# kotakondo/Intent-MPC

Hardware: AMD Instinct MI355X
Metric: QP-solves/s + p50 solve latency, N=20 horizon, batch=65536, 1/2/4/8 MI355X (higher is better)
Workload: dtype f64

## Files before the change

intent-mpc_amd/csrc/impc_qp.hip:

```cpp
#include <hip/hip_runtime.h>
#include <hipcub/hipcub.hpp>

#include <algorithm>
#include <cstdio>
#include <cstring>
#include <memory>
#include <string>
#include <type_traits>
#include <vector>

#include "../../include/impc_qp.h"
#include "../../include/impc_select.h"
#include "../../include/impc_mpc.h"
#include "../../include/impc_fanout.h"
#include "../../include/impc_predict.h"
#include "../../include/impc_detect.h"
#include "../../include/impc_comm.h"
#include "../../include/impc_replan.h"
#include "lib_internal.hpp"
#include "mpc_qp_internal.hpp"
#include "admm_core.hpp"
#include "mpc_structure.hpp"
#include "mpc_wave.hpp"
#include "queue.hpp"
// ... 115 lines not shown
        double qj = IMPC_AT(wk.q, j);
        if (st.scaling > 0) {
            qj = IMPC_AT(wk.D, j) * qj;
            qj *= c;
        }
        IMPC_AT(wk.qs, j) = qj;
    }
}

__global__ __launch_bounds__(kBlock) void k_update_bounds(impc::DevSym sy, impc::DevWork wk, impc::DevSettings st,
                                                          int64_t B) {
    const int lane = blockIdx.x * kBlock + threadIdx.x;
    if (lane >= B) return;
    const int64_t S = wk.S;
    const double rho = IMPC_AT(wk.scal, impc::SC_RHO);
    int changed = 0;
    for (int32_t i = 0; i < sy.m; i++) {
        double li = impc::dmin(impc::dmax(IMPC_AT(wk.l, i), -impc::kInf), impc::kInf);
        double ui = impc::dmin(impc::dmax(IMPC_AT(wk.u, i), -impc::kInf), impc::kInf);
        if (st.scaling > 0) {
            li = IMPC_AT(wk.E, i) * li;
            ui = IMPC_AT(wk.E, i) * ui;
        }
        IMPC_AT(wk.ls, i) = li;
        IMPC_AT(wk.us, i) = ui;
        double t, r;
        if ((li < -impc::kInf * impc::kMinScaling) && (ui > impc::kInf * impc::kMinScaling)) {
            t = -1.0;
            r = impc::kRhoMin;
        } else if (ui - li < impc::kRhoTol) {
            t = 1.0;
            r = rho * impc::kRhoEqOverIneq;
        } else {
            t = 0.0;
            r = rho;
        }
        if (IMPC_AT(wk.ctype, i) != t) {
            IMPC_AT(wk.ctype, i) = t;
            IMPC_AT(wk.rho, i) = r;
            IMPC_AT(wk.rhoinv, i) = 1. / r;
            changed = 1;
        }
    }
    if (changed) {
        int bad = impc::assemble_and_factor(sy, wk, st, lane);
        if (bad) IMPC_AT(wk.scal, impc::SC_SETUP_ERR) = (double)IMPC_NONCVX_ERROR;
    }
    impc::refresh_v(sy, wk, lane);
}

#ifndef IMPC_LCOMB
#define IMPC_LCOMB 1
#endif
template <int NL>
struct GpuTeam {
    double *red;
    __device__ int lane() const { return (int)threadIdx.x; }
    __device__ static void wave_sync() {
        __builtin_amdgcn_fence(__ATOMIC_ACQ_REL, "wavefront");
        __builtin_amdgcn_wave_barrier();
    }
    __device__ void sync() {
        if constexpr (NL == 64) wave_sync();
        else __syncthreads();
    }
    __device__ static void wsync() { wave_sync(); }
    __device__ void lsync() { sync(); }
    __device__ double bcast(double v, int src) {
        int lo = __builtin_amdgcn_readlane(__double2loint(v), src);
        int hi = __builtin_amdgcn_readlane(__double2hiint(v), src);
        return __hiloint2double(hi, lo);
    }
    __device__ static double uniform(double v) {
        int lo = __builtin_amdgcn_readfirstlane(__double2loint(v));
        int hi = __builtin_amdgcn_readfirstlane(__double2hiint(v));
        return __hiloint2double(hi, lo);
    }
    __device__ double shfl(double v, int src) {
        const int addr = src << 2;
        int lo = __builtin_amdgcn_ds_bpermute(addr, __double2loint(v));
        int hi = __builtin_amdgcn_ds_bpermute(addr, __double2hiint(v));
        return __hiloint2double(hi, lo);
    }
    template <int CTRL>
    __device__ static double dpp(double v) {
        int lo = __builtin_amdgcn_mov_dpp(__double2loint(v), CTRL, 0xF, 0xF, true);
        int hi = __builtin_amdgcn_mov_dpp(__double2hiint(v), CTRL, 0xF, 0xF, true);
        return __hiloint2double(hi, lo);
    }
    template <bool ODD>
    __device__ static double mfma_step(double f, double c, double v) {
        const double d = __builtin_amdgcn_mfma_f64_4x4x4f64(f, v, c, 0, 0, 0);
        return d + dpp<ODD ? 0x128 : 0x141>(d);
    }
    __device__ double sum_contig8(double v) {
        v = v + dpp<0xB1>(v);
        v = v + dpp<0x4E>(v);
        v = v + dpp<0x141>(v);
        return v;
    }
    __device__ static double add_dup(double x, double y) {
        double r;
        asm("v_add_f64 %0, %1, %2" : "=v"(r) : "v"(x), "v"(y));
        return r;
    }
    template <bool P32, bool DUP>
    __device__ static double pair_sum2(double a, double b, double *dup) {
        const int al = __double2loint(a), ah = __double2hiint(a), bl = __double2loint(b), bh = __double2hiint(b);
        auto rl = P32 ? __builtin_amdgcn_permlane32_swap(al, bl, false, false)
                      : __builtin_amdgcn_permlane16_swap(al, bl, false, false);
        auto rh = P32 ? __builtin_amdgcn_permlane32_swap(ah, bh, false, false)
                      : __builtin_amdgcn_permlane16_swap(ah, bh, false, false);
        const double x = __hiloint2double(rh[0], rl[0]), y = __hiloint2double(rh[1], rl[1]);
        if (DUP) *dup = add_dup(x, y);
        return x + y;
    }
    __device__ double sum_stride8(double v) {
        const double d = dpp<0x128>(v);
        const double a = v + d, b = add_dup(v, d);
        double c2;
        const double c = pair_sum2<false, true>(a, b, &c2);
        return pair_sum2<true, false>(c, c2, nullptr);
    }
    __device__ static double xor4(double v) {
        const int lo = __builtin_amdgcn_ds_swizzle(__double2loint(v), (4 << 10) | 0x1F);
        const int hi = __builtin_amdgcn_ds_swizzle(__double2hiint(v), (4 << 10) | 0x1F);
        return __hiloint2double(hi, lo);
    }
    __device__ double max(double v) {
        double mv[1] = {v};
        reduce<1, 0>(mv, nullptr);
        return mv[0];
    }
    template <int K>
    __device__ void max_n(double (&v)[K]) {
        reduce<K, 0>(v, nullptr);
    }
    template <int KM, int KS>
    __device__ void max_sum_n(double (&mx)[KM], double (&sm)[KS]) {
        reduce<KM, KS>(mx, sm);
    }
    template <bool P32>
    __device__ static void swap64(double &x, double &y) {
        const int xl = __double2loint(x), xh = __double2hiint(x), yl = __double2loint(y), yh = __double2hiint(y);
        auto rl = P32 ? __builtin_amdgcn_permlane32_swap(xl, yl, false, false)
                      : __builtin_amdgcn_permlane16_swap(xl, yl, false, false);
        auto rh = P32 ? __builtin_amdgcn_permlane32_swap(xh, yh, false, false)
                      : __builtin_amdgcn_permlane16_swap(xh, yh, false, false);
        x = __hiloint2double(rh[0], rl[0]);
        y = __hiloint2double(rh[1], rl[1]);
    }
    template <int KM, int KS>
    __device__ void reduce(double (&mx)[KM], double *sm) {
        constexpr int K1 = (KM + 1) / 2, K2 = (K1 + 1) / 2, KT = KM + KS;
        static_assert(KT * (NL / 64) <= impc::kRedLen, "team reduction scratch (WaveLds RED_OFF)");
        auto vmax = [](double a, double b) { return b > a ? b : a; };
        double h[K1], q[K2];
        _Pragma("unroll") for (int k = 0; k < K1; k++) {
            double x = mx[k], y = k + K1 < KM ? mx[k + K1] : mx[k];
            swap64<true>(x, y);
            h[k] = vmax(x, y);
        }
        _Pragma("unroll") for (int k = 0; k < K2; k++) {
            double x = h[k], y = k + K2 < K1 ? h[k + K2] : h[k];
            swap64<false>(x, y);
            double t = vmax(x, y);
            t = vmax(t, dpp<0xB1>(t));
            t = vmax(t, dpp<0x4E>(t));
            t = vmax(t, dpp<0x141>(t));
            q[k] = vmax(t, dpp<0x128>(t));
        }
        _Pragma("unroll") for (int k = 0; k < KS; k++) sm[k] = wave_sum(sm[k]);
        const int w = (int)threadIdx.x >> 6, row = ((int)threadIdx.x >> 4) & 3;
        if ((threadIdx.x & 15) == 0) {
            _Pragma("unroll") for (int k = 0; k < K2; k++) {
                const int sub = (row & 1) * K2 + k, idx = (row >> 1) * K1 + sub;
                if (sub < K1 && idx < KM) red[w * KT + idx] = q[k];
            }
        }
        if ((threadIdx.x & 63) == 0) _Pragma("unroll") for (int k = 0; k < KS; k++) red[w * KT + KM + k] = sm[k];
        __syncthreads();
#if IMPC_LCOMB
        if constexpr (NL > 64) {
            static_assert(KT <= 64, "one lane per reduced value");
            const int l = (int)threadIdx.x & 63, k = l < KT ? l : 0;
            double r = red[k];
            for (int u = 1; u < NL / 64; u++) {
                const double o = red[u * KT + k];
                const double m = vmax(r, o), a = r + o;
                r = k < KM ? m : a;
            }
            _Pragma("unroll") for (int j = 0; j < KM; j++) mx[j] = bcast(r, j);
            _Pragma("unroll") for (int j = 0; j < KS; j++) sm[j] = bcast(r, KM + j);
            __syncthreads();
            return;
        }
#endif
        _Pragma("unroll") for (int k = 0; k < KM; k++) {
            double r = red[k];
            for (int u = 1; u < NL / 64; u++) r = vmax(r, red[u * KT + k]);
            mx[k] = r;
        }
        _Pragma("unroll") for (int k = 0; k < KS; k++) {
            double r = red[KM + k];
            for (int u = 1; u < NL / 64; u++) r = r + red[u * KT + KM + k];
            sm[k] = r;
        }
        __syncthreads();
    }
    __device__ double wave_sum(double v) {
        {
            const int lo = __double2loint(v), hi = __double2hiint(v);
            auto ql = __builtin_amdgcn_permlane32_swap(lo, lo, false, false);
            auto qh = __builtin_amdgcn_permlane32_swap(hi, hi, false, false);
            v = __hiloint2double(qh[0], ql[0]) + __hiloint2double(qh[1], ql[1]);
        }
        {
            const int lo = __double2loint(v), hi = __double2hiint(v);
            auto rl = __builtin_amdgcn_permlane16_swap(lo, lo, false, false);
            auto rh = __builtin_amdgcn_permlane16_swap(hi, hi, false, false);
            v = __hiloint2double(rh[0], rl[0]) + __hiloint2double(rh[1], rl[1]);
        }
        v = v + dpp<0x128>(v);
        v = v + xor4(v);
        v = v + dpp<0x4E>(v);
        v = v + dpp<0xB1>(v);
        return v;
    }
    __device__ double sum(double v) {
        v = wave_sum(v);
        v = bcast(v, 0);
        if (NL == 64) return v;
        if ((threadIdx.x & 63) == 0) red[threadIdx.x >> 6] = v;
        __syncthreads();
        double r = red[0];
        for (int w = 1; w < NL / 64; w++) r = r + red[w];
        __syncthreads();
        return r;
    }
};

struct GroupEntry {
    impc::WaveTables T;
    impc::WaveIO io;
    impc::DevSettings st;
    int64_t first;
    const int64_t *dcount;
};

template <int NL, int VS, int GS, int WPS, int WF, bool TIER>
__global__ __launch_bounds__(NL, WPS) void k_mpc_wave_group(const GroupEntry *__restrict__ g, int count,
                                                            int64_t total, unsigned *counter,
                                                            const uint32_t *__restrict__ ord, int devcnt) {
    extern __shared__ __attribute__((aligned(16))) double smem[];
    using LD = impc::WaveLds<NL, VS, GS>;
    GpuTeam<NL> wv{smem + LD::RED_OFF};
    __shared__ unsigned next;
    int cur = -1;
    if (devcnt) {
        int64_t t = 0;
        for (int e = 0; e < count; e++) {
            const int64_t c = g[e].dcount ? *g[e].dcount : g[e].io.B;
            t += c < g[e].io.B ? (c > 0 ? c : 0) : g[e].io.B;
        }
        total = t;
    }
    for (;;) {
        if (threadIdx.x == 0) next = atomicAdd(counter, 1u);
        __syncthreads();
        const unsigned pos = next;
        __syncthreads();
        if ((int64_t)pos >= total) break;
        const unsigned b = ord ? ord[pos] : pos;
        int e = 0;
        while (e + 1 < count && (int64_t)b >= g[e + 1].first) e++;
        if (e != cur) {
            impc::WaveQP<GpuTeam<NL>, NL, VS, GS, WF, TIER>::load_tables(wv, g[e].T, smem);
            cur = e;
        }
        impc::WaveQP<GpuTeam<NL>, NL, VS, GS, WF, TIER> qp(wv, g[e].T, g[e].io, g[e].st, smem);
        qp.solve((int64_t)b - g[e].first);
    }
}

}

struct impc_ctx_s {
    int device = 0;
    int num_cu = 256;
    hipStream_t stream = nullptr;
    double tick_s = 1e-8;
    struct GroupTable {
        GroupEntry *d = nullptr;
        int cap = 0;
        std::vector<GroupEntry> h;
        uint64_t used = 0;
    };
    std::vector<GroupTable> groups;
    uint64_t group_clock = 0;
    hipEvent_t ev_order = nullptr;
    std::vector<hipEvent_t> ev_pool, ev_pending;
    std::vector<hipEvent_t> timer_marks;
    std::vector<std::pair<uint64_t, impc_batch_s *>> pool;
};

static int h2d_sync(hipStream_t st, void *dst, const void *src, size_t bytes) {
    if (!bytes) return IMPC_OK;
    HIP_OK(hipMemcpyAsync(dst, src, bytes, hipMemcpyHostToDevice, st));
    HIP_OK(hipStreamSynchronize(st));
    return IMPC_OK;
}
static int fill0_sync(hipStream_t st, void *dst, size_t bytes) {
    if (!bytes) return IMPC_OK;
    HIP_OK(hipMemsetAsync(dst, 0, bytes, st));
    HIP_OK(hipStreamSynchronize(st));
    return IMPC_OK;
}
#define IMPC_TRY(expr)          \
    do {                        \
        int rc_ = (expr);       \
        if (rc_) return rc_;    \
    } while (0)

static int ctx_order_launch(impc_ctx ctx, hipStream_t st) {
    if (st == ctx->stream) return IMPC_OK;
    if (!ctx->ev_order) HIP_OK(hipEventCreateWithFlags(&ctx->ev_order, hipEventDisableTiming));
    HIP_OK(hipEventRecord(ctx->ev_order, ctx->stream));
    HIP_OK(hipStreamWaitEvent(st, ctx->ev_order, 0));
    return IMPC_OK;
}
static int ctx_order_after_all(impc_ctx ctx, hipStream_t st) {
    if (st != ctx->stream) IMPC_TRY(ctx_order_launch(ctx, st));
    for (hipEvent_t e : ctx->ev_pending) HIP_OK(hipStreamWaitEvent(st, e, 0));
// ... 1970 lines not shown
```

intent-mpc_amd/csrc/mpc_wave.hpp:

```cpp
#pragma once
#include <hip/hip_runtime.h>
#include <math.h>
#include <stdint.h>

#include "../../include/impc_qp.h"
#include "admm_core.hpp"
#include "mpc_structure.hpp"
#include "sweep_mfma_map.hpp"

namespace impc {

#define IMPC_WF __host__ __device__ __forceinline__

#ifndef IMPC_PRIO
#define IMPC_PRIO 2
#endif
#if IMPC_PRIO && defined(__HIP_DEVICE_COMPILE__)
#define IMPC_PRIO_UP() __builtin_amdgcn_s_setprio(IMPC_PRIO)
#define IMPC_PRIO_DOWN() __builtin_amdgcn_s_setprio(0)
#else
#define IMPC_PRIO_UP() ((void)0)
#define IMPC_PRIO_DOWN() ((void)0)
#endif
#ifndef IMPC_SWEEP_MFMA
// ... 48 lines not shown

struct WaveTables {
    int32_t n, m, mg, N, W, CG, nnzP, nnzA;
    const int32_t *var_orig, *var_pdiag, *var_boxrow, *var_boxpos;
    const int32_t *gen_row, *gen_col, *gen_pos, *colg, *term_ptr, *term;
    int32_t HS;
    const int32_t *col_hid;
    int32_t T1r;
    int32_t scal_lds;
};

struct WaveIO {
    int64_t B;
    const double *Px, *q, *Ax, *l, *u, *xws, *yws;
    int32_t has_ws;
    double *xo, *yo;
    double *scal;
    impc_info *info;
    unsigned long long *sec = nullptr;
    unsigned long long *qpt = nullptr;
    int32_t shared = 0;
    int64_t nvar = 0;
    const int32_t *vmap = nullptr;
    const double *Ax_var = nullptr;
    double *persist = nullptr;
    int32_t resume = 0, q_updated = 0;
    const double *tlim = nullptr;
    const double *q_scale = nullptr;
};

constexpr int kPersistHdr = 24;
constexpr int kPersistMaxScaling = 20;
IMPC_HD int64_t persist_stride(int n, int mg) { return kPersistHdr + 3 * (int64_t)n + 2 * (int64_t)mg; }

enum {
    kSecSetup, kSecFactor, kSecWarm, kSecRhs, kSecS1, kSecFwd, kSecS3, kSecBwd, kSecS5, kSecUpdate, kSecProducts,
    kSecChecks, kSecOutput, kSecFAsm, kSecFDense, kSecIters = 15, kSecCount = 16
};
#if defined(IMPC_SECTION_PROF) && defined(__HIP_DEVICE_COMPILE__)
#define IMPC_SEC_CLOCK() ((uint64_t)__builtin_amdgcn_s_memrealtime())
#define IMPC_SEC(X)                             \
    do {                                        \
        uint64_t t_ = IMPC_SEC_CLOCK();         \
        sec_acc[X] += t_ - sec_t0;              \
        sec_t0 = t_;                            \
    } while (0)
#define IMPC_SEC_START() (sec_t0 = IMPC_SEC_CLOCK())
#else
#define IMPC_SEC(X) ((void)0)
#define IMPC_SEC_START() ((void)0)
#endif

constexpr int kRedLen = 128;

template <int NL, int VS, int GS>
struct WaveLds {
    static constexpr int NMAX = NL * VS;
    static constexpr int WMAX = (NMAX + 5) / 13 - 1;
    static constexpr int WSPEC = NMAX <= 256 ? 19 : 39;
    static constexpr int WSPEC2 = NMAX <= 256 ? 0 : 29;
    static constexpr int NP = (NMAX + 48 > (779 + NMAX + 3) / 4) ? NMAX + 48 : (779 + NMAX + 3) / 4;
    static constexpr int F_OFF = 0;
    static constexpr int R_OFF = F_OFF + WMAX * 64;
    static constexpr int T_OFF = R_OFF + NP;
    static constexpr int E_OFF = T_OFF + NP;
    static constexpr int X_OFF = E_OFF + NP;
    static constexpr int RED_OFF = X_OFF + NP;
    static constexpr int JUNK_OFF = RED_OFF + kRedLen;
    static constexpr int GSLOT_OFF = JUNK_OFF + NL;
    static constexpr bool ONCHIP = VS == 1;
    static constexpr int VEC_N = 2 * NMAX + NL * GS;
    static constexpr int SCL_OFF = GSLOT_OFF + NL * GS;
    static constexpr int DLT_OFF = SCL_OFF + (ONCHIP ? VEC_N : 0);
    static constexpr int DLT_N = ONCHIP && GS > 2 ? NL * (GS - 2) : 0;
    static constexpr int P_OFF = DLT_OFF + DLT_N;
    static constexpr int CGM = 24;
    static constexpr int T1 = kProdTier1;
    static IMPC_WF int cg4(int CG) { return (CG + 3) & ~3; }
    static constexpr IMPC_WF int stride(int n) { return ((n + 63) & ~63) + 1; }
    static IMPC_WF int hsp(int HS) { return HS + 1; }
    static IMPC_WF int p_size(int CG, int n, int HS, int mg, int T1r) {
        const int c = T1r * stride(n) + (cg4(CG) > T1r ? (cg4(CG) - T1r) * hsp(HS) : 0), f = 5 * mg;
        return c > f ? c : f;
    }
    static IMPC_WF int p_size(const WaveTables &T) { return p_size(T.CG, T.n, T.HS, T.mg, T.T1r); }
    static constexpr int CHX = (VS == 1 && IMPC_CHUNK19) ? 448 : 0;
    static IMPC_WF int ch_off(const WaveTables &T) { return P_OFF + p_size(T) + 8; }
    static IMPC_WF int scl2_off(const WaveTables &T) { return P_OFF + p_size(T) + 8 + CHX; }
    static IMPC_WF int size(const WaveTables &T) {
        return scl2_off(T) + (!ONCHIP && T.scal_lds ? 2 * T.n + T.mg : 0);
    }
    static constexpr int FA = R_OFF, FL = FA + 169, FI = FL + 169, FB = FI + 169, FG = FB + 104, FE = FG + 104,
                         DIAGX = FE + 64;
    static_assert(DIAGX + NMAX <= RED_OFF, "factorisation scratch does not fit");
    static constexpr int FB2 = DIAGX + NMAX;
    static_assert(VS != 3 || FB2 + 104 <= RED_OFF, "factorisation scratch does not fit");
};

constexpr int64_t kRefailMark = -1000;

struct WaveRho {
    double rho, r_eq, r_ineq, r_loose, i_eq, i_ineq, i_loose;
    IMPC_WF void set(double r) {
        rho = r;
        r_ineq = r;
        r_eq = kRhoEqOverIneq * r;
        r_loose = kRhoMin;
        i_ineq = 1. / r_ineq;
        i_eq = 1. / r_eq;
        i_loose = 1. / r_loose;
    }
    IMPC_WF double of(int t) const {
        double e = t > 0 ? 1.0 : 0.0, i = t == 0 ? 1.0 : 0.0, l = t < 0 ? 1.0 : 0.0;
        return (e * r_eq + i * r_ineq) + l * r_loose;
    }
    IMPC_WF double inv(int t) const {
        double e = t > 0 ? 1.0 : 0.0, i = t == 0 ? 1.0 : 0.0, l = t < 0 ? 1.0 : 0.0;
        return (e * i_eq + i * i_ineq) + l * i_loose;
    }
};

IMPC_WF int row_type(double l, double u) {
    if ((l < -kInf * kMinScaling) && (u > kInf * kMinScaling)) return -1;
    if (u - l < kRhoTol) return 1;
    return 0;
}

template <class WV, int NL, int VS, int GS, int WF = 0, bool TIER = false>
struct WaveQP {
    using LD = WaveLds<NL, VS, GS>;
    static_assert(WF == 0 || WF == LD::WSPEC || WF == LD::WSPEC2, "WF is 0 or one of the shape's compiled horizons");
    IMPC_WF int Wst() const { return WF ? WF : T.W; }
    WV &wv;
    const WaveTables &T;
    const WaveIO &io;
    const DevSettings &st;
    double *lds;
    int L;
    double x[VS], q[VS], pd[VS], ab[VS], zb[VS], yb[VS], lb[VS], ub[VS], dxv_[VS], dyb_[VS];
    double ainv[VS][13], cp[VS][8];
    int bt[VS], vs_[VS], vr_[VS], hid_[VS];
    bool vok[VS];
    double a[GS][4], z[GS], y[GS], lg[GS], ug[GS], dyg_[GS];
    int gc[GS][4], gt[GS];
    bool gok[GS];
    WaveRho R;
    double c = 1.0, cinv = 1.0;
    int rw = 0;
    double sig_, alp_;
    int c4_, sd_;
#if defined(IMPC_SECTION_PROF) && defined(__HIP_DEVICE_COMPILE__)
    uint64_t sec_t0 = 0, sec_acc[kSecCount] = {};
#endif

    IMPC_WF WaveQP(WV &w, const WaveTables &t, const WaveIO &i, const DevSettings &s, double *l)
        : wv(w), T(t), io(i), st(s), lds(l), L(w.lane()), sig_(s.sigma), alp_(s.alpha), c4_(LD::cg4(t.CG)),
          sd_(LD::stride(t.n)) {}

    IMPC_WF int lane_o() const {
        int l = L;
#if defined(__HIP_DEVICE_COMPILE__)
        asm volatile("" : "+v"(l));
#endif
        return l;
    }

    IMPC_WF static void opaque(int &v) {
#if defined(__HIP_DEVICE_COMPILE__)
        asm volatile("" : "+v"(v));
#else
        (void)v;
#endif
    }

    IMPC_WF void set_rho(double r) { R.set(wv.uniform(r)); }
    IMPC_WF double rhob(int s) const { return R.of(bt[s]); }
    IMPC_WF double rhoib(int s) const { return R.inv(bt[s]); }
    IMPC_WF double rhog_(int s) const { return R.of(gt[s]); }
    IMPC_WF double rhoig_(int s) const { return R.inv(gt[s]); }

    IMPC_WF double &dxv(int s) {
        if constexpr (LD::ONCHIP) return lds[LD::JUNK_OFF + NL * s + L]; else return dxv_[s];
    }
    IMPC_WF double &dyb(int s) { if constexpr (LD::ONCHIP) return lds[LD::R_OFF + NL * s + L]; else return dyb_[s]; }
    IMPC_WF double &dyg(int s) {
        if constexpr (LD::ONCHIP)
            return lds[(s == 0 ? LD::T_OFF : s == 1 ? LD::E_OFF : LD::DLT_OFF + NL * (s - 2)) + L];
        else
            return dyg_[s];
    }
    IMPC_WF double *scal(int64_t b) {
        if constexpr (LD::ONCHIP) return lds + LD::SCL_OFF;
        else return T.scal_lds ? lds + LD::scl2_off(T) : io.scal + b * (int64_t)(2 * T.n + T.mg);
    }

    IMPC_WF double *F() { return lds + LD::F_OFF; }
    IMPC_WF double *rbuf() { return lds + LD::R_OFF; }
    IMPC_WF double *tbuf() { return lds + LD::T_OFF; }
    IMPC_WF double *ebuf() { return lds + LD::E_OFF; }
    IMPC_WF double *xbuf() { return lds + LD::X_OFF; }
    IMPC_WF double *pbuf() { return lds + LD::P_OFF; }

    static constexpr bool F3 = IMPC_FACT2 && IMPC_FACT3 && VS == 3;
    static constexpr int NCH = (WF > 0 && VS == 3 && IMPC_CHUNK5) ? 5 : 4;
    static constexpr bool CHUNK = WF > 0 && NL == 256 && (VS == 3 || (VS == 1 && IMPC_CHUNK19 != 0));
    static constexpr int CL = WF > 0 ? (NCH == 5 ? 2 * ((WF + 9) / 10) : 2 * ((WF + 7) / 8)) : 2;
    static constexpr int CLAST = WF - (NCH - 1) * CL;
    static constexpr int CH_OFF = LD::F_OFF + 64 * (WF + 3);
    enum { kChFP1 = 0, kChFP2 = 64, kChFP21 = 128, kChBT1 = 192, kChBT2 = 256, kChBT21 = 320 };
    enum { kCh5P1 = 0, kCh5P2 = 64, kCh5P3 = 128, kCh5P21 = 192, kCh5P32 = 256, kCh5P321 = 320, kCh5B = 384 };
    static constexpr int kChEnd = NCH == 5 ? 768 : 384;
    static constexpr int kChEnds = NCH == 5 ? 24 : 16;
    static_assert(!CHUNK || VS == 1 || CH_OFF + kChEnd + 2 * kChEnds <= LD::R_OFF,
                  "chunk operators do not fit the F region");
    static_assert(!CHUNK || VS != 1 || LD::CHX >= kChEnd + 2 * kChEnds, "chunk operator region");
    IMPC_WF double *chbuf() const { return lds + (VS == 1 ? LD::ch_off(T) : CH_OFF); }
    static_assert(!CHUNK || (CLAST >= 1 && CLAST <= CL), "chunk lengths");

    IMPC_WF void clear_exchange() {
        for (int i = L; i < 4 * LD::NP; i += NL) lds[LD::R_OFF + i] = 0.0;
        wv.sync();
    }

    IMPC_WF void load(int64_t b) {
        const int n = T.n, m = T.m;
        const int64_t bn = b * n, bm = b * m, bP = io.shared ? 0 : b * T.nnzP, bA = io.shared ? 0 : b * T.nnzA;
        auto Aval = [&](int p) -> double {
            if (io.shared) {
                const int32_t v = io.vmap[p];
                return v >= 0 ? io.Ax_var[b * io.nvar + v] : io.Ax[p];
            }
            return io.Ax[bA + p];
// ... 59 lines not shown
            if (id >= 0)
                gs[id] = (int16_t)(t < T.T1r ? t * LD::stride(T.n) + v
                                             : T.T1r * LD::stride(T.n) + (t - T.T1r) * LD::hsp(T.HS) + T.col_hid[v]);
        }
        w.sync();
    }

    IMPC_WF void zero_products() {
        double *pb = pbuf();
        const int cnt = LD::p_size(T) + 8;
        for (int i = L; i < cnt; i += NL) pb[i] = 0.0;
        wv.sync();
    }

    IMPC_WF int gcol(int s, int e) const { return gc[s][e] & 0xFFFF; }
    IMPC_WF int gdst(int s, int e) const { return gc[s][e] >> 16; }

    template <int NG>
    IMPC_WF static double gather_n(const double *pb, int sd) {
        double p[4 * NG];
        _Pragma("unroll") for (int t = 0; t < 4 * NG; t++) p[t] = pb[t * sd];
        double s = 0.0;
        _Pragma("unroll") for (int g = 0; g < NG; g++) s += (p[4 * g] + p[4 * g + 1]) + (p[4 * g + 2] + p[4 * g + 3]);
        return s;
    }

    IMPC_WF double col_gather(int v, int h) {
        const double *pb = pbuf() + v;
        const int C4 = c4_, sd = WF ? LD::stride(13 * (WF + 1) - 5) : sd_;
        double s = 0.0;
        if constexpr (!TIER) {
            (void)h;
            switch (C4) {
                case 4: return gather_n<1>(pb, sd);
                case 8: return gather_n<2>(pb, sd);
                case 12: return gather_n<3>(pb, sd);
                case 16: return gather_n<4>(pb, sd);
                case 20: return gather_n<5>(pb, sd);
                default: break;
            }
            for (int t = 0; t < C4; t += 4) {
                const double p0 = pb[t * sd], p1 = pb[(t + 1) * sd], p2 = pb[(t + 2) * sd], p3 = pb[(t + 3) * sd];
                s += (p0 + p1) + (p2 + p3);
            }
        } else {
            static_assert(LD::T1 == 4, "one first-tier group");
            s += (pb[0] + pb[sd]) + (pb[2 * sd] + pb[3 * sd]);
            if (h >= 0) {
                const int hp = LD::hsp(T.HS);
                const double *q = pbuf() + LD::T1 * sd + h;
                for (int t = 0; t < C4 - LD::T1; t += 4)
                    s += (q[t * hp] + q[(t + 1) * hp]) + (q[(t + 2) * hp] + q[(t + 3) * hp]);
            }
        }
        return s;
    }
    IMPC_WF double col_gather_max(int v, int h) {
        const double *pb = pbuf() + v;
        const int C4 = c4_, sd = sd_;
        double s = 0.0;
        for (int t = 0; t < (TIER ? LD::T1 : C4); t++) s = dmax(pb[t * sd], s);
        if (TIER && h >= 0) {
            const int hp = LD::hsp(T.HS);
            const double *q = pbuf() + LD::T1 * sd + h;
            for (int t = 0; t < C4 - LD::T1; t++) s = dmax(q[t * hp], s);
        }
        return s;
    }

    IMPC_WF void scale(int64_t b, double D[VS], double Eb[VS], double Eg[GS], double *ps) {
        const int n = T.n;
        _Pragma("unroll") for (int s = 0; s < VS; s++) D[s] = Eb[s] = 1.0;
        _Pragma("unroll") for (int s = 0; s < GS; s++) Eg[s] = 1.0;
        c = 1.0;
        double *pb = pbuf(), *xb = xbuf();
#if IMPC_FACT2
        if (st.scaling > 0) {
            _Pragma("unroll") for (int s = 0; s < GS; s++) {
                if (gok[s])
                    _Pragma("unroll") for (int e = 0; e < 4; e++) pb[gdst(s, e)] = fabs(a[s][e]);
            }
            wv.sync();
        }
#endif
        for (int it = 0; it < st.scaling; it++) {
#if !IMPC_FACT2
            _Pragma("unroll") for (int s = 0; s < GS; s++) {
                if (gok[s])
                    _Pragma("unroll") for (int e = 0; e < 4; e++) pb[gdst(s, e)] = fabs(a[s][e]);
            }
            wv.sync();
#endif
            double Dt[VS], Etb[VS], Etg[GS];
            _Pragma("unroll") for (int s = 0; s < VS; s++) {
                double d = fabs(pd[s]);
                double an = dmax(fabs(ab[s]), 0.0);
                if (vok[s]) an = dmax(col_gather_max(NL * s + L, hid_[s]), an);
                d = dmax(d, an);
                d = d < kMinScaling ? 1.0 : d;
                d = d > kMaxScaling ? kMaxScaling : d;
                Dt[s] = 1.0 / sqrt(d);
                double e = fabs(ab[s]);
                e = e < kMinScaling ? 1.0 : e;
                e = e > kMaxScaling ? kMaxScaling : e;
                Etb[s] = 1.0 / sqrt(e);
            }
// ... 697 lines not shown
        }
        wv.lsync();
        if (w == 1) {
            (void)fwd_run<CL, true>(tb, rb, CL, rb[A1 + i]);
        } else if (w == 2) {
            const double a = wv.sum_contig8(__builtin_fma(C[kCh5P1 + l], rb[A1 + j], 0.125 * ends[i]));
            (void)fwd_run<CL, true>(tb, rb, 2 * CL, a);
        } else if (w == 3) {
            const double p = __builtin_fma(C[kCh5P2 + l], ends[j],
                                           __builtin_fma(C[kCh5P21 + l], rb[A1 + j], 0.125 * ends[8 + i]));
            (void)fwd_run<CL, true>(tb, rb, 3 * CL, wv.sum_contig8(p));
        } else {
            const double p = __builtin_fma(
                C[kCh5P3 + l], ends[8 + j],
                __builtin_fma(C[kCh5P32 + l], ends[j], __builtin_fma(C[kCh5P321 + l], rb[A1 + j], 0.125 * ends[16 + i])));
            (void)fwd_run<CLAST, true>(tb, rb, 4 * CL, wv.sum_contig8(p));
        }
    }

    IMPC_WF void bwd_chunked5(const double *eb, double *xb) {
        const double *C = chbuf() + kCh5B;
        double *ends = chbuf() + kChEnd + kChEnds;
        const int w = L >> 6, l = lane_o() & 63, i = l >> 3, j = l & 7;
        constexpr int X4 = 13 * 4 * CL;
        constexpr bool LODD = (WF - 1) & 1;
        if (w == 0) {
            (void)bwd_run<LODD, CLAST, true>(eb, xb, 4 * CL, 8.0 * eb[13 * WF + (LODD ? i : j)]);
        } else {
            const double e = bwd_run<true, CL, false>(eb, xb, (4 - w) * CL, 0.0);
            if (j == 0) ends[8 * (w - 1) + i] = e;
        }
        wv.lsync();
        if (w == 1) {
            (void)bwd_run<true, CL, true>(eb, xb, 3 * CL, xb[X4 + i]);
        } else if (w == 2) {
            const double x = wv.sum_contig8(__builtin_fma(C[kCh5P1 + l], xb[X4 + j], 0.125 * ends[i]));
            (void)bwd_run<true, CL, true>(eb, xb, 2 * CL, x);
        } else if (w == 3) {
            const double p = __builtin_fma(C[kCh5P2 + l], ends[j],
                                           __builtin_fma(C[kCh5P21 + l], xb[X4 + j], 0.125 * ends[8 + i]));
            (void)bwd_run<true, CL, true>(eb, xb, CL, wv.sum_contig8(p));
        } else {
            const double p = __builtin_fma(
                C[kCh5P3 + l], ends[8 + j],
                __builtin_fma(C[kCh5P32 + l], ends[j], __builtin_fma(C[kCh5P321 + l], xb[X4 + j], 0.125 * ends[16 + i])));
            (void)bwd_run<true, CL, true>(eb, xb, 0, wv.sum_contig8(p));
        }
    }

    IMPC_WF void write_v_products() {
        double *pb = pbuf();
        _Pragma("unroll") for (int s = 0; s < GS; s++) {
            double vv = rhog_(s) * z[s] - y[s];
            _Pragma("unroll") for (int e = 0; e < 4; e++) pb[gdst(s, e)] = a[s][e] * vv;
        }
        wv.lsync();
    }

    IMPC_WF void iterate(bool need_delta) {
        const int W = Wst();
        double *rb = rbuf(), *tb = tbuf(), *eb = ebuf(), *xb = xbuf();
        const double sigma = sig_;
        IMPC_REP(kSecRhs) {
            _Pragma("unroll") for (int s = 0; s < VS; s++) {
                int v = NL * s + L;
                double vb = rhob(s) * zb[s] - yb[s];
                double r = sigma * x[s] - q[s];
                r += ab[s] * vb;
                r += col_gather(v, hid_[s]);
                rb[v] = r;
            }
            wv.lsync();
        }
        IMPC_SEC(kSecRhs);
        IMPC_REP(kSecS1) {
            _Pragma("unroll") for (int s = 0; s < VS; s++) {
                int v = NL * s + L;
                double t = rb[v];
                const double *rp = lds + (vs_[s] > 0 ? LD::R_OFF + 13 * (vs_[s] - 1) + 8 : LD::X_OFF + LD::NMAX);
                double rv[5];
                _Pragma("unroll") for (int cc = 0; cc < 5; cc++) rv[cc] = rp[cc];
                IMPC_LOADS_FIRST(5, 12);
                _Pragma("unroll") for (int cc = 0; cc < 5; cc++) t -= cp[s][cc] * rv[cc];
                tb[v] = kSweepPre * t;
            }
            wv.lsync();
        }
        IMPC_SEC(kSecS1);
        IMPC_REP(kSecFwd) {
            if constexpr (CHUNK && NCH == 5) {
                fwd_chunked5(tb, rb);
            } else if constexpr (CHUNK) {
                fwd_chunked(tb, rb);
            } else if ((L >> 6) == rw) {
                IMPC_PRIO_UP();
                if (W == LD::WSPEC)
                    fwd_sweep<LD::WSPEC>(tb, rb, W);
                else
                    fwd_sweep<0>(tb, rb, W);
                IMPC_PRIO_DOWN();
            }
            wv.lsync();
        }
        IMPC_SEC(kSecFwd);
        IMPC_REP(kSecS3) {
            _Pragma("unroll") for (int s = 0; s < VS; s++) {
                const double *rk = lds + LD::R_OFF + 13 * vs_[s];
                double rv[13];
                _Pragma("unroll") for (int cc = 0; cc < 13; cc++) rv[cc] = rk[cc];
                IMPC_LOADS_FIRST(7, 20);
                double e = 0.0;
                _Pragma("unroll") for (int cc = 0; cc < 13; cc++) e += ainv[s][cc] * rv[cc];
                eb[NL * s + L] = vr_[s] < 8 ? kSweepPre * e : e;
            }
            wv.lsync();
        }
        IMPC_SEC(kSecS3);
        IMPC_REP(kSecBwd) {
            if (L < 8) xb[13 * W + L] = (1.0 / kSweepPre) * eb[13 * W + L];
            if constexpr (CHUNK && NCH == 5) {
                bwd_chunked5(eb, xb);
            } else if constexpr (CHUNK) {
                bwd_chunked(eb, xb);
            } else if ((L >> 6) == rw) {
                IMPC_PRIO_UP();
                if (W == LD::WSPEC)
                    bwd_sweep<((LD::WSPEC - 1) & 1) != 0, LD::WSPEC>(eb, xb, W);
                else if ((W - 1) & 1)
                    bwd_sweep<true, 0>(eb, xb, W);
                else
                    bwd_sweep<false, 0>(eb, xb, W);
                IMPC_PRIO_DOWN();
            }
            wv.lsync();
        }
        IMPC_SEC(kSecBwd);
        IMPC_REP(kSecS5) {
            _Pragma("unroll") for (int s = 0; s < VS; s++) {
                const double *xn = lds + LD::X_OFF + 13 * (vs_[s] + 1);
                double t = eb[NL * s + L];
                double xv[8];
                _Pragma("unroll") for (int j = 0; j < 8; j++) xv[j] = xn[j];
                IMPC_LOADS_FIRST(5, 16);
                _Pragma("unroll") for (int j = 0; j < 8; j++) t -= cp[s][j] * xv[j];
                *(vok[s] && vr_[s] >= 8 ? xb + NL * s + L : lds + LD::JUNK_OFF + L) = t;
            }
            wv.lsync();
        }
        IMPC_SEC(kSecS5);
        update_and_products(need_delta);
    }

    IMPC_WF static double clampz(double v, double l, double u) { return __builtin_fmin(__builtin_fmax(v, l), u); }

    IMPC_WF void update_and_products(bool need_delta) {
        double *xb = xbuf();
        const double alpha = alp_, oma = (double)1.0 - alp_;
        _Pragma("unroll") for (int s = 0; s < VS; s++) {
            if (!vok[s]) continue;
            double xt = xb[NL * s + L];
            double xn = alpha * xt + oma * x[s];
            if (need_delta) dxv(s) = xn - x[s];
            x[s] = xn;
            double zt = ab[s] * xt;
            double zr = alpha * zt + oma * zb[s];
            double zn = clampz(zr + rhoib(s) * yb[s], lb[s], ub[s]);
            double dy = rhob(s) * (zr - zn);
            yb[s] += dy;
            if (need_delta) dyb(s) = dy;
            zb[s] = zn;
        }
        double xg[GS][4];
        _Pragma("unroll") for (int s = 0; s < GS; s++) {
            _Pragma("unroll") for (int e = 0; e < 4; e++) xg[s][e] = xb[gcol(s, e)];
        }
        IMPC_LOADS_FIRST(4 * GS, 8 * GS);
        _Pragma("unroll") for (int s = 0; s < GS; s++) {
            double zt = 0.0;
            _Pragma("unroll") for (int e = 0; e < 4; e++) zt += a[s][e] * xg[s][e];
            double zr = alpha * zt + oma * z[s];
            double zn = clampz(zr + rhoig_(s) * y[s], lg[s], ug[s]);
            double dy = rhog_(s) * (zr - zn);
            y[s] += dy;
            if (need_delta) dyg(s) = dy;
            z[s] = zn;
        }
        IMPC_SEC(kSecUpdate);
        IMPC_REP(kSecProducts) write_v_products();
        IMPC_SEC(kSecProducts);
    }

    struct Info {
        double pri_res, dua_res, pri_norm_u, dua_norm_u, pri_norm_s, dua_norm_s, pri_plain, dua_plain;
        double pinf_nrm, pinf_lhs, dinf_nrm, dinf_qdx, dinf_pdx;
    };

    IMPC_WF void load_scal(int64_t b, double D[VS], double Eb[VS], double Eg[GS]) {
        const double *sc = scal(b);
        _Pragma("unroll") for (int s = 0; s < VS; s++) {
            D[s] = vok[s] ? sc[NL * s + L] : 1.0;
            Eb[s] = vok[s] ? sc[T.n + NL * s + L] : 1.0;
        }
        _Pragma("unroll") for (int s = 0; s < GS; s++) Eg[s] = gok[s] ? sc[2 * T.n + NL * s + L] : 1.0;
    }

    IMPC_WF void update_info(Info &inf, const double D[VS], const double Eb[VS], const double Eg[GS]) {
        const bool unsc = st.scaling > 0 && !st.scaled_termination;
        double *xb = xbuf(), *pb = pbuf();
        _Pragma("unroll") for (int s = 0; s < VS; s++)
            if (vok[s]) xb[NL * s + L] = x[s];
        _Pragma("unroll") for (int s = 0; s < GS; s++) {
            if (gok[s])
                _Pragma("unroll") for (int e = 0; e < 4; e++) pb[gdst(s, e)] = a[s][e] * y[s];
        }
        wv.sync();
        double pr_u = 0, z_u = 0, ax_u = 0, pr_p = 0, z_p = 0, ax_p = 0;
        _Pragma("unroll") for (int s = 0; s < VS; s++) {
            if (!vok[s]) continue;
            double ax = ab[s] * x[s], r = ax + -1 * zb[s], ei = 1. / Eb[s];
            pr_p = dmax(pr_p, fabs(r));
            z_p = dmax(z_p, fabs(zb[s]));
            ax_p = dmax(ax_p, fabs(ax));
            pr_u = dmax(pr_u, fabs(ei * r));
            z_u = dmax(z_u, fabs(ei * zb[s]));
            ax_u = dmax(ax_u, fabs(ei * ax));
        }
        _Pragma("unroll") for (int s = 0; s < GS; s++) {
            if (!gok[s]) continue;
            double ax = 0.0;
            _Pragma("unroll") for (int e = 0; e < 4; e++) ax += a[s][e] * xb[gcol(s, e)];
            double r = ax + -1 * z[s], ei = 1. / Eg[s];
            pr_p = dmax(pr_p, fabs(r));
            z_p = dmax(z_p, fabs(z[s]));
            ax_p = dmax(ax_p, fabs(ax));
// ... 312 lines not shown
                y[s] = yv;
                double zz = 0.0;
                _Pragma("unroll") for (int e = 0; e < 4; e++) zz += a[s][e] * xb[gcol(s, e)];
                z[s] = zz;
            }
            wv.sync();
            clear_exchange();
        }
        write_v_products();
        IMPC_SEC(kSecWarm);

        int64_t status = IMPC_UNSOLVED, rho_updates = 0;
        int32_t iter;
        double obj = 0.0, rho_est = R.rho;
        Info inf{};
        int64_t info_iter = 0;
        const int chk = st.check_termination;
        int can_check = 0;
        int32_t max_iter = st.max_iter;
        const int32_t rho_int = st.adaptive_rho ? st.rho_interval : 0;
        const double tl = wv.uniform(io.tlim ? io.tlim[b] : st.time_limit), tick = st.tick_s;
        const bool tlim = tl > 0;
        int32_t chk_left = chk, rho_left = rho_int;
        bool refac = false;
        iter = 1;
        for (;;) {
            if (refac) {
                refac = false;
                const bool last = LD::ONCHIP && iter > max_iter;
                double kdy[VS], kdg[GS];
                if (last) {
                    _Pragma("unroll") for (int s = 0; s < VS; s++) kdy[s] = vok[s] ? dyb(s) : 0.0;
                    _Pragma("unroll") for (int s = 0; s < GS; s++) kdg[s] = gok[s] ? dyg(s) : 0.0;
                }
                if (factorize()) {
                    max_iter = 0;
                    status = kRefailMark;
                }
                if (last) {
                    _Pragma("unroll") for (int s = 0; s < VS; s++)
                        if (vok[s]) dyb(s) = kdy[s];
                    _Pragma("unroll") for (int s = 0; s < GS; s++) dyg(s) = kdg[s];
                }
                write_v_products();
                IMPC_SEC(kSecFactor);
            }
            bool chk_now = false, rho_now = false, stop = false;
            if (iter <= max_iter) {
                int nxt = max_iter - iter + 1;
                if (chk && chk_left < nxt) nxt = chk_left;
                if (rho_int && rho_left < nxt) nxt = rho_left;
                const bool ce = chk && chk_left == nxt, re = rho_int && rho_left == nxt;
                const bool nd_last = ce || iter + nxt - 1 == max_iter || tlim;
                for (int t = 1;; t++) {
                    iterate(t == nxt ? nd_last : tlim);
                    if (tlim) {
                        const double el = wv.max((double)(device_clock() - t0) * tick);
                        if (el >= tl) {
                            status = IMPC_TIME_LIMIT_REACHED;
                            stop = true;
                            if (t > 1) can_check = 0;
                            break;
                        }
                    }
                    if (t == nxt) break;
                    iter++;
                }
                if (!stop) {
                    chk_now = ce;
                    rho_now = re;
                    if (chk) chk_left = ce ? chk : chk_left - nxt;
                    if (rho_int) rho_left = re ? rho_int : rho_left - nxt;
                    can_check = chk_now;
                    if (!(chk_now || rho_now)) iter++;
                }
            }
            if (stop || iter > max_iter) break;
            if (can_check) {
                IMPC_SEC_START();
                double D[VS], Eb[VS], Eg[GS];
                load_scal(b, D, Eb, Eg);
                int done = 0;
                IMPC_REP(kSecChecks) {
                    update_info(inf, D, Eb, Eg);
                    done = check_termination(inf, 0, status, obj, D, Eb, Eg);
                }
                info_iter = iter;
                write_v_products();
                IMPC_SEC(kSecChecks);
                if (done) break;
            }
            if (rho_now) {
                if (!can_check) {
                    double D[VS], Eb[VS], Eg[GS];
                    load_scal(b, D, Eb, Eg);
                    update_info(inf, D, Eb, Eg);
                    info_iter = iter;
                    write_v_products();
                }
                double rn = rho_estimate(inf);
                rho_est = rn;
                if ((rn > R.rho * st.adaptive_rho_tolerance) || (rn < R.rho / st.adaptive_rho_tolerance)) {
                    IMPC_SEC(kSecChecks);
                    set_rho(dmin(dmax(rn, kRhoMin), kRhoMax));
                    rho_updates += 1;
                    refac = true;
// ... 90 lines not shown
```

Before: 381,700.

## Add dense-occupancy WaveQP variant with LDS rho table and register-pressure barriers

Adds a DENSE template variant, used when waves-per-SIMD exceeds the shape default, that keeps the rho and inverse-rho values in a small LDS table and snapshots the bounds and linear-term registers once per iteration pass. Empty asm barriers and raw v_max/v_min clamps stop the compiler from rematerializing or spreading these values, and packed gather indices replace separate gcol/gdst lookups. The aim is to cut VGPR pressure so more waves fit per SIMD. In exchange it adds LDS reads and a sync in set_rho, and the asm barriers may block useful compiler optimizations.

```diff
diff --git a/intent-mpc_amd/csrc/impc_qp.hip b/intent-mpc_amd/csrc/impc_qp.hip
--- a/intent-mpc_amd/csrc/impc_qp.hip
+++ b/intent-mpc_amd/csrc/impc_qp.hip
@@ -191,7 +191,7 @@
 #ifndef IMPC_LCOMB
 #define IMPC_LCOMB 1
 #endif
-template <int NL>
+template <int NL, bool LEAN = false>
 struct GpuTeam {
     double *red;
     __device__ int lane() const { return (int)threadIdx.x; }
@@ -292,7 +292,7 @@
     template <int KM, int KS>
     __device__ void reduce(double (&mx)[KM], double *sm) {
         constexpr int K1 = (KM + 1) / 2, K2 = (K1 + 1) / 2, KT = KM + KS;
-        static_assert(KT * (NL / 64) <= impc::kRedLen, "team reduction scratch (WaveLds RED_OFF)");
+        static_assert(KT * (NL / 64) <= impc::kRedUsed, "team reduction scratch (WaveLds RED_OFF)");
         auto vmax = [](double a, double b) { return b > a ? b : a; };
         double h[K1], q[K2];
         _Pragma("unroll") for (int k = 0; k < K1; k++) {
@@ -310,7 +310,9 @@
             q[k] = vmax(t, dpp<0x128>(t));
         }
         _Pragma("unroll") for (int k = 0; k < KS; k++) sm[k] = wave_sum(sm[k]);
-        const int w = (int)threadIdx.x >> 6, row = ((int)threadIdx.x >> 4) & 3;
+        int tid = (int)threadIdx.x;
+        if constexpr (LEAN) asm volatile("" : "+v"(tid));
+        const int w = tid >> 6, row = (tid >> 4) & 3;
         if ((threadIdx.x & 15) == 0) {
             _Pragma("unroll") for (int k = 0; k < K2; k++) {
                 const int sub = (row & 1) * K2 + k, idx = (row >> 1) * K1 + sub;
@@ -393,7 +395,10 @@
                                                             const uint32_t *__restrict__ ord, int devcnt) {
     extern __shared__ __attribute__((aligned(16))) double smem[];
     using LD = impc::WaveLds<NL, VS, GS>;
-    GpuTeam<NL> wv{smem + LD::RED_OFF};
+    constexpr bool DENSE = WPS > Shape<VS>::WPS;
+    using TEAM = GpuTeam<NL, DENSE>;
+    using QP = impc::WaveQP<TEAM, NL, VS, GS, WF, TIER, DENSE>;
+    TEAM wv{smem + LD::RED_OFF};
     __shared__ unsigned next;
     int cur = -1;
     if (devcnt) {
@@ -414,10 +419,10 @@
         int e = 0;
         while (e + 1 < count && (int64_t)b >= g[e + 1].first) e++;
         if (e != cur) {
-            impc::WaveQP<GpuTeam<NL>, NL, VS, GS, WF, TIER>::load_tables(wv, g[e].T, smem);
+            QP::load_tables(wv, g[e].T, smem);
             cur = e;
         }
-        impc::WaveQP<GpuTeam<NL>, NL, VS, GS, WF, TIER> qp(wv, g[e].T, g[e].io, g[e].st, smem);
+        QP qp(wv, g[e].T, g[e].io, g[e].st, smem);
         qp.solve((int64_t)b - g[e].first);
     }
 }
diff --git a/intent-mpc_amd/csrc/mpc_wave.hpp b/intent-mpc_amd/csrc/mpc_wave.hpp
--- a/intent-mpc_amd/csrc/mpc_wave.hpp
+++ b/intent-mpc_amd/csrc/mpc_wave.hpp
@@ -124,6 +124,7 @@
 #endif
 
 constexpr int kRedLen = 128;
+constexpr int kRedUsed = kRedLen - 8;
 
 template <int NL, int VS, int GS>
 struct WaveLds {
@@ -198,7 +199,7 @@
     return 0;
 }
 
-template <class WV, int NL, int VS, int GS, int WF = 0, bool TIER = false>
+template <class WV, int NL, int VS, int GS, int WF = 0, bool TIER = false, bool DENSE = false>
 struct WaveQP {
     using LD = WaveLds<NL, VS, GS>;
     static_assert(WF == 0 || WF == LD::WSPEC || WF == LD::WSPEC2, "WF is 0 or one of the shape's compiled horizons");
@@ -245,11 +246,70 @@
 #endif
     }
 
-    IMPC_WF void set_rho(double r) { R.set(wv.uniform(r)); }
-    IMPC_WF double rhob(int s) const { return R.of(bt[s]); }
-    IMPC_WF double rhoib(int s) const { return R.inv(bt[s]); }
-    IMPC_WF double rhog_(int s) const { return R.of(gt[s]); }
-    IMPC_WF double rhoig_(int s) const { return R.inv(gt[s]); }
+    static constexpr int kRhoTab = LD::RED_OFF + kRedUsed;
+    IMPC_WF void set_rho(double r) {
+        R.set(wv.uniform(r));
+        if constexpr (DENSE) {
+            if (L == 0) {
+                double *t = lds + kRhoTab;
+                t[0] = R.r_loose, t[1] = R.r_ineq, t[2] = R.r_eq;
+                t[3] = R.i_loose, t[4] = R.i_ineq, t[5] = R.i_eq;
+            }
+            wv.lsync();
+        }
+    }
+    IMPC_WF double rho_of(int t) const {
+        if constexpr (DENSE) return lds[kRhoTab + 1 + t]; else return R.of(t);
+    }
+    IMPC_WF double rho_inv(int t) const {
+        if constexpr (DENSE) return lds[kRhoTab + 4 + t]; else return R.inv(t);
+    }
+    IMPC_WF double rhob(int s) const { return rho_of(bt[s]); }
+    IMPC_WF double rhoib(int s) const { return rho_inv(bt[s]); }
+    IMPC_WF double rhog_(int s) const { return rho_of(gt[s]); }
+    IMPC_WF double rhoig_(int s) const { return rho_inv(gt[s]); }
+
+    struct Pass {
+        double lb[VS], ub[VS], lg[GS], ug[GS], q[VS];
+        int hq[VS];
+        int hp;
+    } ps_;
+    IMPC_WF static void opaque(double &v) {
+#if defined(__HIP_DEVICE_COMPILE__)
+        asm volatile("" : "+v"(v));
+#else
+        (void)v;
+#endif
+    }
+    IMPC_WF void begin_pass() {
+        if constexpr (DENSE) {
+            static_assert(!DENSE || (TIER && WF > 0), "the denser instance is the two-tier default horizon's");
+            auto own = [](double v) {
+                opaque(v);
+                return v;
+            };
+            _Pragma("unroll") for (int s = 0; s < VS; s++) {
+                ps_.lb[s] = own(lb[s]);
+                ps_.ub[s] = own(ub[s]);
+                ps_.q[s] = own(q[s]);
+                ps_.hq[s] = hid_[s] >= 0 ? LD::T1 * LD::stride(13 * (WF + 1) - 5) + hid_[s] : -1;
+                opaque(ps_.hq[s]);
+            }
+            _Pragma("unroll") for (int s = 0; s < GS; s++) {
+                ps_.lg[s] = own(lg[s]);
+                ps_.ug[s] = own(ug[s]);
+            }
+            ps_.hp = LD::hsp(T.HS);
+#if defined(__HIP_DEVICE_COMPILE__)
+            asm volatile("" : "+s"(ps_.hp));
+#endif
+        }
+    }
+    IMPC_WF int gpk(int s, int e) const {
+        int g = gc[s][e];
+        if (DENSE && s == GS - 1 && e == 3) opaque(g);
+        return g;
+    }
 
     IMPC_WF double &dxv(int s) {
         if constexpr (LD::ONCHIP) return lds[LD::JUNK_OFF + NL * s + L]; else return dxv_[s];
@@ -415,6 +475,20 @@
                 for (int t = 0; t < C4 - LD::T1; t += 4)
                     s += (q[t * hp] + q[(t + 1) * hp]) + (q[(t + 2) * hp] + q[(t + 3) * hp]);
             }
+        }
+        return s;
+    }
+    IMPC_WF double col_gather_pass(int v, int slot) {
+        static_assert(LD::T1 == 4, "one first-tier group");
+        const double *pb = pbuf() + v;
+        constexpr int sd = LD::stride(13 * (WF + 1) - 5);
+        double s = 0.0;
+        s += (pb[0] + pb[sd]) + (pb[2 * sd] + pb[3 * sd]);
+        if (ps_.hq[slot] >= 0) {
+            const int hp = ps_.hp;
+            const double *q = pbuf() + ps_.hq[slot];
+            for (int t = 0; t < c4_ - LD::T1; t += 4)
+                s += (q[t * hp] + q[(t + 1) * hp]) + (q[(t + 2) * hp] + q[(t + 3) * hp]);
         }
         return s;
     }
@@ -1218,7 +1292,7 @@
         double *pb = pbuf();
         _Pragma("unroll") for (int s = 0; s < GS; s++) {
             double vv = rhog_(s) * z[s] - y[s];
-            _Pragma("unroll") for (int e = 0; e < 4; e++) pb[gdst(s, e)] = a[s][e] * vv;
+            _Pragma("unroll") for (int e = 0; e < 4; e++) pb[gpk(s, e) >> 16] = a[s][e] * vv;
         }
         wv.lsync();
     }
@@ -1231,9 +1305,9 @@
             _Pragma("unroll") for (int s = 0; s < VS; s++) {
                 int v = NL * s + L;
                 double vb = rhob(s) * zb[s] - yb[s];
-                double r = sigma * x[s] - q[s];
+                double r = sigma * x[s] - (DENSE ? ps_.q[s] : q[s]);
                 r += ab[s] * vb;
-                r += col_gather(v, hid_[s]);
+                if constexpr (DENSE) r += col_gather_pass(v, s); else r += col_gather(v, hid_[s]);
                 rb[v] = r;
             }
             wv.lsync();
@@ -1318,6 +1392,16 @@
     }
 
     IMPC_WF static double clampz(double v, double l, double u) { return __builtin_fmin(__builtin_fmax(v, l), u); }
+    IMPC_WF static double clampz_raw(double v, double l, double u) {
+#if defined(__HIP_DEVICE_COMPILE__)
+        double r;
+        asm("v_max_f64 %0, %1, %2" : "=v"(r) : "v"(v), "v"(l));
+        asm("v_min_f64 %0, %1, %2" : "=v"(r) : "v"(r), "v"(u));
+        return r;
+#else
+        return clampz(v, l, u);
+#endif
+    }
 
     IMPC_WF void update_and_products(bool need_delta) {
         double *xb = xbuf();
@@ -1330,7 +1414,9 @@
             x[s] = xn;
             double zt = ab[s] * xt;
             double zr = alpha * zt + oma * zb[s];
-            double zn = clampz(zr + rhoib(s) * yb[s], lb[s], ub[s]);
+            double zn;
+            if constexpr (DENSE) zn = clampz_raw(zr + rhoib(s) * yb[s], ps_.lb[s], ps_.ub[s]);
+            else zn = clampz(zr + rhoib(s) * yb[s], lb[s], ub[s]);
             double dy = rhob(s) * (zr - zn);
             yb[s] += dy;
             if (need_delta) dyb(s) = dy;
@@ -1338,14 +1424,16 @@
         }
         double xg[GS][4];
         _Pragma("unroll") for (int s = 0; s < GS; s++) {
-            _Pragma("unroll") for (int e = 0; e < 4; e++) xg[s][e] = xb[gcol(s, e)];
+            _Pragma("unroll") for (int e = 0; e < 4; e++) xg[s][e] = xb[gpk(s, e) & 0xFFFF];
         }
         IMPC_LOADS_FIRST(4 * GS, 8 * GS);
         _Pragma("unroll") for (int s = 0; s < GS; s++) {
             double zt = 0.0;
             _Pragma("unroll") for (int e = 0; e < 4; e++) zt += a[s][e] * xg[s][e];
             double zr = alpha * zt + oma * z[s];
-            double zn = clampz(zr + rhoig_(s) * y[s], lg[s], ug[s]);
+            double zn;
+            if constexpr (DENSE) zn = clampz_raw(zr + rhoig_(s) * y[s], ps_.lg[s], ps_.ug[s]);
+            else zn = clampz(zr + rhoig_(s) * y[s], lg[s], ug[s]);
             double dy = rhog_(s) * (zr - zn);
             y[s] += dy;
             if (need_delta) dyg(s) = dy;
@@ -1764,6 +1852,7 @@
                 if (rho_int && rho_left < nxt) nxt = rho_left;
                 const bool ce = chk && chk_left == nxt, re = rho_int && rho_left == nxt;
                 const bool nd_last = ce || iter + nxt - 1 == max_iter || tlim;
+                begin_pass();
                 for (int t = 1;; t++) {
                     iterate(t == nxt ? nd_last : tlim);
                     if (tlim) {
```

After: 435,400 (median of 6 runs). 14.1% higher.
